# jakewendt/ghostm

Hardware: AMD Instinct MI355X
Metric: query residues aligned/sec (whole node) + bit-identical hit-list vs CPU (higher is better)
Workload: dtype int (exact 16-bit integers; packed f16 max3 orders their patterns, no guard)

## Files before the change

ghostm_amd/csrc/device.hip:

```cpp
#include <hip/hip_runtime.h>

#include <algorithm>
#include <atomic>
#include <climits>
#include <cstdio>
#include <cstdlib>
#include <cstring>
#include <mutex>
#include <string>
#include <vector>

#include "../../include/ghostm_hip.h"
#include "band_align.h"
#include "frame_align.h"
#include "common.h"
#include "device.h"
#include "formats.h"
#include "hit_batches.h"
#include "index.h"
#include "kernels.h"
#include "path_rows.h"
#include "read_rows.h"
#include "read_pileup.h"
#include "pileup_plan.h"
// ... 185 lines not shown
  DevBuf subj;
  DevBuf subj_bucket;
  uint32_t nsubj = 0;
};

struct DeviceModule::Impl {
  int h_matrix[32 * 32] = {0};
  static constexpr int kStageSlots = 4;
  static constexpr size_t kStagePiece = 8u << 20;
  PinnedBuf stage[kStageSlots];
  hipEvent_t stage_ev[kStageSlots] = {};
  bool stage_busy[kStageSlots] = {};
  int stage_turn = 0;
  DevBuf mat_k2, mat_tb, mat_tbk;
  DevBuf mat_raw;
  DevBuf counts, nelem, slots, offsets, qlist, gbuf, gbuf_off, list_beg, list_len;
  DevBuf cand_start, cand_qid;
  DevBuf records, rec_prefix;
  std::vector<uint32_t> h_rec_prefix;
  uint64_t ncand = 0;
  DevBuf task_buf[2], tasks_redo, score_out, end_out, guard_list;
  int task_turn = 0;
  struct Prepared {
    bool valid = false;
    uint64_t cand_begin = 0, n = 0;
    uint32_t count = 0, per_block = 0;
    bool swar = false;
    int kind = kScoreRows;
    int buf = 0;
  } prepared;
  struct ScoreState {
    bool active = false, guarded = false;
    uint64_t cand_begin = 0, n = 0;
    size_t lds = 0;
    int S = 32;
    kern::ScoreArgs args{};
  } score_state;
  struct DeferredNext {
    bool valid = false;
    DeviceModule::ScoreSegment seg{};
    bool swar = false, pairs_ok = true;
    uint32_t per_block = 0;
    size_t bytes = 0;
    uint32_t sparse_per_block = 0;
  } deferred;
  DevBuf tb_qid, tb_end, tb_start, tb_ml;
  DevBuf tb_ext;
  DevBuf tb_path_in, tb_path_meta, tb_path_dir, tb_path_ops, tb_path_cmp;
  DevBuf path_rows_hit, path_rows_ops, path_rows_out, path_rows_buf;
  DevBuf read_rows_hit, read_rows_ops, read_rows_out, read_rows_buf;
  DevBuf pileup_hit, pileup_ops, pileup_list, pileup_part, pileup_prof, pileup_out, pileup_cols;
  DevBuf band_hit, band_meta, band_dir, band_ops, band_cmp;
  DevBuf frame_hit, frame_meta, frame_dir, frame_ops, frame_cmp;
  DevBuf tb_width, tb_ncols, tb_skey, tb_key, tb_order1, tb_order2, tb_sort, tb_pair_a, tb_pair_b, tb_best;
  int cus = 256;
  DevBuf keys, sel_count, sel_score, sel_sid, slot_hits, sel_from;
  struct MergeState {
    bool active = false;
    uint32_t ng = 0;
// ... 57 lines not shown
  out->data = p;
  out->n = n;
}

DeviceModule &DeviceModule::Get() {
  static DeviceModule *m = new DeviceModule();
  return *m;
}

void DeviceModule::Use() const {
  thread_local int current = -1;
  if (device_ >= 0 && current != device_) {
    HIP_CHECK(hipSetDevice(device_));
    current = device_;
  }
}

void DeviceModule::Bind(int device) {
  if (device_ == device && impl_) {
    Use();
    return;
  }
  if (impl_ && device_ >= 0)
    throw Error("the device module is bound to device " + std::to_string(device_) + "; one device per process");
  int n = 0;
  HIP_CHECK(hipGetDeviceCount(&n));
  if (n <= 0) throw Error("no HIP device visible");
  if (device < 0 || device >= n) throw Error("device id " + std::to_string(device) + " out of range");
  HIP_CHECK(hipSetDevice(device));
  if (!impl_) impl_ = new Impl();
// ... 58 lines not shown
  HIP_CHECK(hipFuncSetAttribute((const void *)kern::k_tb_scan<SS, true, EE, true, true, true>, \
                                hipFuncAttributeMaxDynamicSharedMemorySize, (int)kScanLdsPriv));
  GHOSTM_SCAN_ATTRP(32, true) GHOSTM_SCAN_ATTRP(32, false) GHOSTM_SCAN_ATTRP(16, true)
  GHOSTM_SCAN_ATTRP(16, false) GHOSTM_SCAN_ATTRP(8, true) GHOSTM_SCAN_ATTRP(8, false)
#undef GHOSTM_SCAN_ATTRP
  for (const void *f : {(const void *)kern::k_score_pair<32>, (const void *)kern::k_score_pair<16>,
                        (const void *)kern::k_score_pair<8>})
    HIP_CHECK(hipFuncSetAttribute(f, hipFuncAttributeMaxDynamicSharedMemorySize, (int)(kern::kPairK2Words * 4)));
#undef GHOSTM_SCAN_ATTR2
#undef GHOSTM_SCAN_ATTR
  {
    hipDeviceProp_t p;
    HIP_CHECK(hipGetDeviceProperties(&p, device));
    impl_->cus = p.multiProcessorCount > 0 ? p.multiProcessorCount : 256;
  }
  device_ = device;
}

static hipStream_t S(void *s) { return static_cast<hipStream_t>(s); }

std::string DeviceModule::DeviceName() const {
  hipDeviceProp_t p;
  HIP_CHECK(hipGetDeviceProperties(&p, device_ < 0 ? 0 : device_));
  return std::string(p.name) + " (" + p.gcnArchName + ")";
}

size_t DeviceModule::TotalMemory() const {
  hipDeviceProp_t p;
  HIP_CHECK(hipGetDeviceProperties(&p, device_ < 0 ? 0 : device_));
  return p.totalGlobalMem;
// ... 21 lines not shown
        const int v = q == (int)kern::kPadCode ? -lim - 1 : std::max(-lim, std::min(lim, m[c * 32 + q]));
        tbk[w][c * 32 + q] =
            (int)(((uint32_t)v << (mlw + 2)) | (2u << mlw) | 0x80u | (c == q ? 1u : 0u));
      }
    }
  }
  impl_->mat_raw.Reserve(sizeof(impl_->h_matrix));
  HIP_CHECK(hipMemcpy(impl_->mat_raw.p, impl_->h_matrix, sizeof(impl_->h_matrix), hipMemcpyHostToDevice));
  impl_->mat_k2.Reserve(sizeof(k2));
  impl_->mat_tb.Reserve(sizeof(tb));
  impl_->mat_tbk.Reserve(sizeof(tbk));
  HIP_CHECK(hipMemcpy(impl_->mat_k2.p, k2, sizeof(k2), hipMemcpyHostToDevice));
  HIP_CHECK(hipMemcpy(impl_->mat_tb.p, tb, sizeof(tb), hipMemcpyHostToDevice));
  HIP_CHECK(hipMemcpy(impl_->mat_tbk.p, tbk, sizeof(tbk), hipMemcpyHostToDevice));
  impl_->matrix_set = true;
}

void DeviceModule::SetHostCopy(HostCopyFn fn) { host_copy_ = std::move(fn); }
void DeviceModule::SetHostParallel(HostParallelFn fn) { host_par_ = std::move(fn); }

void DeviceModule::StagedUpload(void *dst, const void *src, size_t bytes) {
  Impl &I = *impl_;
  if (bytes < (1u << 20) || !host_copy_) {
    if (bytes) HIP_CHECK(hipMemcpyAsync(dst, src, bytes, hipMemcpyHostToDevice, S(stream_)));
    if (bytes) HIP_CHECK(hipStreamSynchronize(S(stream_)));
    return;
  }
  for (size_t off = 0; off < bytes; off += Impl::kStagePiece) {
    const size_t n = std::min(Impl::kStagePiece, bytes - off);
    const int k = I.stage_turn;
// ... 822 lines not shown
  const bool framed = half && sigma_max <= 1000 && !(force && strcmp(force, "f16plain") == 0);
  const int64_t swar_low = 1024 + 64 + (-(int64_t)gap.open) + (-(int64_t)gap.ext);
  const int64_t swar_restart = swar_low + sigma_max + bound + 32;
  const int64_t swar_top = swar_restart + sigma_max + bound + std::abs((int64_t)gap.open - gap.ext) + 32;
  const bool swar = framed && swar_top < 0x7C00 && !(force && strcmp(force, "f16frame") == 0);
  const int64_t swar_rise = swar_top - swar_restart;
  const int64_t swar_step = swar_rise + 32;
  const uint64_t max_ends = d->end_gap == UINT32_MAX || base == 0 ? 1 : (uint64_t)(base - 1) / d->end_gap + 1;
  const int64_t swar_cap = swar_restart + (int64_t)(max_ends - 1) * swar_step;
  const char *levels_env = getenv("GHOSTM_K2_LEVELS");
  const bool levels = swar && !(levels_env && strcmp(levels_env, "0") == 0) && max_ends <= 64 && swar_cap + swar_rise < 0x7C00;
  int guard = swar ? 0 : framed ? (bound + sigma_max < 2040 ? 0 : (int)(2040 - sigma_max)) : (bound < 2048 ? 0 : 2000);
  if (half && getenv("GHOSTM_K2_GUARD")) guard = atoi(getenv("GHOSTM_K2_GUARD"));
  const uint32_t per_block = ScorePerBlock(q, d, base, gap);
  const uint32_t sparse_pb = swar ? SparsePerBlock(q, d) : 0u;
  int kind = kScoreRows;
  int buf = -1;
  size_t ntasks = 0;
  auto task_bytes = [&](uint64_t cn, uint32_t q0, uint32_t q1) {
    const uint32_t pb = sparse_pb ? std::min(per_block, sparse_pb) : per_block;
    return std::max<size_t>(ScoreTaskBound(cn, q0, q1, pb, kern::kScoreQmaxUnit) * sizeof(kern::ScoreTask),
                            (size_t)cn * 4);
  };
  if (I.prepared.valid && I.prepared.cand_begin == cand_begin && I.prepared.n == n &&
      I.prepared.per_block == per_block && I.prepared.swar == swar) {
    buf = I.prepared.buf;
    ntasks = I.prepared.count;
    kind = I.prepared.kind;
    HIP_CHECK(hipStreamWaitEvent(S(stream_), I.ev_tasks, 0));
  }
  const bool stale = I.prepared.valid;
  I.prepared.valid = false;
  if (buf < 0) {
    buf = I.task_turn;
    if (stale) HIP_CHECK(hipEventSynchronize(I.ev_tasks));
    PinnedBuf &hs = I.h_tasks[buf];
    hs.Reserve(task_bytes(n, q_first, q_end));
    ntasks = BuildTasks(swar, cand_begin, n, q_first, q_end, counts, offsets, per_block, hs.as<kern::ScoreTask>(),
                        &kind, guard == 0, &host_par_, sparse_pb);
    TraceMark("tasks", ntasks);
    if (const char *dump = getenv("GHOSTM_DEBUG_TASKS")) {
      if (FILE *f = fopen(dump, "ab")) {
        const uint64_t hdr[6] = {cand_begin, n, q_first, q_end, (uint64_t)kind, (uint64_t)ntasks};
        fwrite(hdr, 8, 6, f);
        fwrite(hs.p, kind == kScorePairs ? 4 : sizeof(kern::ScoreTask), ntasks, f);
        fwrite(counts.data() + q_first, 4, q_end - q_first, f);
        fwrite(offsets.data() + q_first, 8, q_end - q_first, f);
        fclose(f);
      }
    }
    const size_t tb = ntasks * (kind == kScorePairs ? 4 : sizeof(kern::ScoreTask));
    I.task_buf[buf].Reserve(tb);
    HIP_CHECK(hipMemcpyAsync(I.task_buf[buf].p, hs.p, tb, hipMemcpyHostToDevice, S(stream_)));
    TraceMark("tasks_up", ntasks);
// ... 28 lines not shown
  a.extend = gap.extend;
  a.open = gap.open;
  a.ext = gap.ext;
  a.score_out = I.score_out.as<uint32_t>();
  a.end_out = I.end_out.as<uint32_t>();
  a.out_base = cand_begin;
  a.swar_low = (uint32_t)swar_low;
  a.swar_restart = (uint32_t)swar_restart;
  a.swar_step = levels ? (uint32_t)swar_step : 0u;
  a.swar_cap = levels ? (uint32_t)swar_cap : 0u;
  if (pairs) {
    a.pairs = I.task_buf[buf].as<uint32_t>();
    a.npairs = (uint32_t)ntasks;
    a.fcodes = q->fcodes.as<uint32_t>();
  }
  if (sparse) {
    a.Lpad = slay.Lpad;
    a.pad = slay.Lpad - q->L;
    a.G = slay.G;
    a.gpw = slay.gpw;
    a.prof_slots = kern::SparseSlots();
    a.prof_rows = kern::kProfRowsSparse;
  }
  I.counters.Reserve(32);
  HIP_CHECK(hipMemsetAsync(I.counters.p, 0, 32, S(stream_)));
  a.cells = I.counters.as<unsigned long long>();
  if (half && guard) {
    I.guard_list.Reserve((size_t)n * 8);
    a.guard = guard;
    a.guard_count = reinterpret_cast<uint32_t *>(I.counters.as<unsigned long long>() + 2);
    a.guard_list = I.guard_list.as<uint32_t>();
  }
  const size_t lds = unit     ? (size_t)kern::kScoreQmaxUnit * kern::kProfRows16 * (lay.Lpad + 4) * 4 + 32 * 32 * 4
                     : sparse ? (size_t)kern::SparseSlots() * kern::kProfRowsSparse * (slay.Lpad + 8) * 2 + 32 * 32 * 2
                     : packed ? (size_t)kern::kScoreQmax * kern::kProfRows16 * (lay.Lpad + 8) * 2 + 32 * 32 * 2
                              : (size_t)kern::kScoreQmax * kern::kProfRows * (lay.Lpad + 4) * 4;
  HIP_CHECK(hipEventRecord(I.ev0, S(stream_)));
  const dim3 grid((uint32_t)ntasks), block(kern::kScoreBlock);
  if (pairs) {
    uint32_t ps = std::min<uint32_t>((uint32_t)lay.S, 16);
    if (const char *e = getenv("GHOSTM_K2_PAIR_S")) ps = (uint32_t)atoi(e);
    const uint32_t pg = ps == 8 || ps == 16 || ps == 32 ? lay.Lpad / ps : 0;
    const Layout play = pg >= 1 && pg <= 16 && pg * ps == lay.Lpad ? Layout{(int)ps, pg, lay.Lpad, 64 / pg} : lay;
    a.G = play.G;
    a.gpw = play.gpw;
    const uint32_t per_wg = (kern::kPairBlock / 64) * play.gpw;
    const dim3 pgrid(std::max<uint32_t>(1, std::min<uint32_t>((uint32_t)I.cus, (uint32_t)((ntasks + per_wg - 1) / per_wg))));
    const dim3 pblock(kern::kPairBlock);
// ... 49 lines not shown
  times_.score_launches_swar += swar ? 1 : 0;
  times_.score_launches_unit += unit ? 1 : 0;
  times_.score_launches_pair += pairs ? 1 : 0;
  times_.score_launches_sparse += sparse ? 1 : 0;
  times_.score_launches_levels += levels && (sparse || (packed && !unit && !pairs)) ? 1 : 0;
  P.active = true;
  P.guarded = half && guard;
  P.cand_begin = cand_begin;
  P.n = n;
  P.lds = lds;
  P.S = lay.S;
  P.args = a;
  I.deferred = Impl::DeferredNext{};
  if (next && next->n) {
    I.deferred = Impl::DeferredNext{true, *next, swar, guard == 0, per_block,
                                    task_bytes(next->n, next->q_first, next->q_end), sparse_pb};
    if (!defer_next_) ScorePrepareNext(counts, offsets);
  }
}

void DeviceModule::ScorePrepareNext(const std::vector<uint32_t> &counts, const std::vector<uint64_t> &offsets) {
  Impl &I = *impl_;
  if (!I.deferred.valid) return;
  const Impl::DeferredNext dn = I.deferred;
  I.deferred.valid = false;
  const ScoreSegment *next = &dn.seg;
  const int nb = I.task_turn;
  PinnedBuf &hs = I.h_tasks[nb];
  int nkind = kScoreRows;
  hs.Reserve(dn.bytes);
  const size_t nt = BuildTasks(dn.swar, next->cand_begin, next->n, next->q_first, next->q_end, counts, offsets,
                               dn.per_block, hs.as<kern::ScoreTask>(), &nkind, dn.pairs_ok, nullptr,
                               dn.sparse_per_block);
  const size_t nbytes = nt * (nkind == kScorePairs ? 4 : sizeof(kern::ScoreTask));
  I.task_buf[nb].Reserve(nbytes);
  HIP_CHECK(hipMemcpyAsync(I.task_buf[nb].p, hs.p, nbytes, hipMemcpyHostToDevice, S(copy_stream_)));
  HIP_CHECK(hipEventRecord(I.ev_tasks, S(copy_stream_)));
  I.prepared = Impl::Prepared{true, next->cand_begin, next->n, (uint32_t)nt, dn.per_block, dn.swar, nkind, nb};
}

bool DeviceModule::ScoreGuarded() const { return impl_ && impl_->score_state.active && impl_->score_state.guarded; }

void DeviceModule::ScoreFinish() {
  Use();
  Impl &I = *impl_;
  Impl::ScoreState &P = I.score_state;
  if (!P.active) return;
  P.active = false;
  SettleSeedTime();
  unsigned long long cells = 0;
  uint32_t nguard = 0;
  HIP_CHECK(hipStreamWaitEvent(S(copy_stream_), I.ev1, 0));
  HIP_CHECK(hipMemcpyAsync(&cells, I.counters.p, 8, hipMemcpyDeviceToHost, S(copy_stream_)));
// ... 1945 lines not shown
```

ghostm_amd/csrc/kernels.h:

```cpp
#pragma once
#include <hip/hip_runtime.h>
#include <stdint.h>

#include <type_traits>

#include "lds_poison.h"
#include "libstdcxx_sort.h"
#include "score_task.h"
#include "seed_lists.h"

namespace ghostm {
namespace kern {

constexpr uint32_t kSeqEnd = 25;
constexpr uint32_t kPadCode = 31;
constexpr int kNeg = -30000;

__device__ inline uint32_t ShiftUp(uint32_t v) {
  return (uint32_t)__builtin_amdgcn_mov_dpp((int)v, 0x138, 0xF, 0xF, true);
}

constexpr uint32_t kMaxLists = 128;
constexpr uint32_t kOverflow = 0xFFFFFFFFu;
#ifndef GHOSTM_K1_SLOT
// ... 1197 lines not shown
  uint32_t base, extend;
  int open, ext;
  uint32_t *score_out;
  uint32_t *end_out;
  unsigned long long out_base;
  unsigned long long *cells;
  int guard;
  uint32_t *guard_count;
  uint32_t *guard_list;
  uint32_t swar_low, swar_restart;
  const uint32_t *pairs;
  uint32_t npairs;
  const uint32_t *fcodes;
  uint32_t prof_slots, prof_rows;
  uint32_t swar_step, swar_cap;
};
__device__ inline uint32_t ProfSlots(const ScoreArgs &a) { return a.prof_slots ? a.prof_slots : (uint32_t)kScoreQmax; }
__device__ inline uint32_t ProfRows(const ScoreArgs &a) { return a.prof_rows ? a.prof_rows : kProfRows16; }

template <int S>
__global__ __launch_bounds__(kScoreBlock) void k_score(ScoreArgs a) {
  GHOSTM_POISON_LDS();
  extern __shared__ __attribute__((aligned(16))) int s_prof[];
  const ScoreTask t = a.tasks[blockIdx.x];
  const uint32_t RS = a.Lpad + 4;

  const uint32_t per_slot = kProfRows * a.Lpad;
  const uint32_t total = t.q_count * per_slot;
  for (uint32_t e = threadIdx.x; e < total; e += kScoreBlock) {
    const uint32_t slot = e / per_slot, rem = e - slot * per_slot;
// ... 246 lines not shown
#pragma unroll
      for (int k = 0; k < 4; ++k) {
        const uint4 v = src[k];
        w[4 * k] = v.x;
        w[4 * k + 1] = v.y;
        w[4 * k + 2] = v.z;
        w[4 * k + 3] = v.w;
      }
    }
#pragma unroll
    for (int c = 0; c < 32; ++c)
      if ((uint32_t)c < nrows) dst[c * RS] = (short)((c & 1) ? w[c >> 1] >> 16 : w[c >> 1]);
  }
}

__device__ __forceinline__ void BuildProfileUnit(const ScoreArgs &a, const ScoreTask &t, uint32_t *s_prof32,
                                                 uint32_t RS) {
  uint32_t *s_enc = s_prof32 + kScoreQmaxUnit * kProfRows16 * RS;
  const int extp = -a.ext;
  const uint32_t drop = (uint32_t)(0x10000u - (a.swar_low - 64u)) & 0xFFFFu;
  for (uint32_t e = threadIdx.x; e < 32 * 32; e += kScoreBlock) {
    const uint32_t q = e >> 5, c = e & 31;
    const int v = c < 25 ? a.mat[c * 32 + q] : 0;
    const uint32_t v16 = c < kSeqEnd ? (uint32_t)(v + extp) & 0xFFFFu : drop;
    s_enc[e] = v16 | 0x10000u;
  }
  __syncthreads();
  const uint32_t rows = t.q_count * a.Lpad;
  for (uint32_t p = threadIdx.x; p < rows; p += kScoreBlock) {
    const uint32_t slot = p / a.Lpad, r = p - slot * a.Lpad;
    uint32_t *dst = s_prof32 + slot * kProfRows16 * RS + r;
    if (r < a.pad) {
#pragma unroll
      for (int c = 0; c < 32; ++c) dst[c * RS] = drop | 0x10000u;
    } else {
      const uint32_t query = slot ? t.q_second : t.q_first;
      const uint32_t q = a.qseq[(size_t)query * a.L + (r - a.pad)];
      const uint4 *src = reinterpret_cast<const uint4 *>(s_enc + q * 32);
#pragma unroll
      for (int k = 0; k < 8; ++k) {
        const uint4 v = src[k];
        dst[(4 * k) * RS] = v.x;
        dst[(4 * k + 1) * RS] = v.y;
        dst[(4 * k + 2) * RS] = v.z;
        dst[(4 * k + 3) * RS] = v.w;
      }
    }
  }
}

template <int S, bool HALF>
__global__ __launch_bounds__(kScoreBlock) void k_score16(ScoreArgs a) {
  GHOSTM_POISON_LDS();
  using C = Cells<HALF>;
  extern __shared__ __attribute__((aligned(16))) short s_prof16[];
  const ScoreTask t = a.tasks[blockIdx.x];
  const uint32_t RS = a.Lpad + 8;

  BuildProfile16<C, false>(a, t, s_prof16, RS);
  __syncthreads();

// ... 134 lines not shown
                                             : 0ull);
}

#ifndef GHOSTM_K2_LAREUSE
#define GHOSTM_K2_LAREUSE 1
#endif
template <int S, bool SWAR = false, bool UNIT = false, bool LEVELS = false>
__global__ __launch_bounds__(kScoreBlock) void k_score16f(ScoreArgs a) {
  GHOSTM_POISON_LDS();
  static_assert(!UNIT || SWAR, "unit-pair words carry integer patterns");
  static_assert(!LEVELS || (SWAR && !UNIT), "restart levels: the 16-bit-row integer-pattern kernel");
  constexpr bool LA = UNIT || LEVELS;
  using C = Cells<true>;
  extern __shared__ __attribute__((aligned(16))) short s_prof16[];
  const ScoreTask t = a.tasks[blockIdx.x];
  const uint32_t RS = UNIT ? a.Lpad + 4 : a.Lpad + 8;
  const int extp = -a.ext;

  if constexpr (UNIT)
    BuildProfileUnit(a, t, reinterpret_cast<uint32_t *>(s_prof16), RS);
  else
    BuildProfile16<C, true, SWAR, LEVELS>(a, t, s_prof16, RS);
  __syncthreads();

  const uint32_t lane = threadIdx.x & 63, wave = threadIdx.x >> 6;
  const uint32_t g = lane / a.G, i = lane - g * a.G;
  const uint32_t pair = wave * a.gpw + g;
  const bool in_group = g < a.gpw;
  const bool vA = in_group && 2 * pair < t.count;
  const bool vB = in_group && 2 * pair + 1 < t.count;
  if (!__builtin_amdgcn_ballot_w64(vA)) return;
  unsigned long long cA = t.begin + 2 * pair, cB = cA + 1;
  uint32_t slotA = 0, slotB = 0, offA = 0, offB = 0, wA = 0, wB = 0;
  if constexpr (UNIT) {
    const uint32_t lA = 2 * pair, lB = lA + 1;
    slotA = vA && lA >= t.count1;
    slotB = vB && lB >= t.count1;
    cA = slotA ? t.begin2 + (lA - t.count1) : t.begin + lA;
    cB = slotB ? t.begin2 + (lB - t.count1) : t.begin + lB;
  }
  if (vA) {
    if constexpr (!UNIT) slotA = a.cand_qid[cA] - t.q_first;
    int o = (int)(a.cand_start[cA] - a.extend);
    offA = o < 0 ? 0u : (uint32_t)o;
    wA = a.base;
    if (offA + wA > a.dblen) wA = a.dblen - offA;
  }
  if (vB) {
    if constexpr (!UNIT) slotB = a.cand_qid[cB] - t.q_first;
    int o = (int)(a.cand_start[cB] - a.extend);
    offB = o < 0 ? 0u : (uint32_t)o;
    wB = a.base;
    if (offB + wB > a.dblen) wB = a.dblen - offB;
  }
  typedef unsigned int u32x4 __attribute__((ext_vector_type(4)));
  typedef __attribute__((address_space(3))) const u32x4 lds_u4;
  const uint32_t lds0 = (uint32_t)(uintptr_t)(__attribute__((address_space(3))) const char *)s_prof16;
  constexpr uint32_t EB = UNIT ? 4 : 2;
  const uint32_t SLOT = (UNIT ? kProfRows16 : ProfRows(a)) * RS;
  const uint32_t baseA2 = lds0 + (slotA * SLOT + i * S) * EB;
  const uint32_t baseB2 = lds0 + (slotB * SLOT + i * S) * EB;
  const uint8_t *dbp = a.db - kDbFrontPad;
  const uint32_t back = kDbFrontPad + a.dblen;
  const uint32_t xA = (vA ? offA + kDbFrontPad : back) - i, xB = (vB ? offB + kDbFrontPad : back) - i;
  const uint32_t RS2 = RS * EB;
  const __amdgpu_buffer_rsrc_t dbr = __builtin_amdgcn_make_buffer_rsrc((void *)dbp, 0, 0x7FFFFFFF, 0x00020000);
  const uint32_t EXTP = SWAR ? (uint32_t)extp * 0x10001u : C::Pair(extp);
  const hf2 KOE = HF(C::Pair(a.open - a.ext));
  const hf2 NEXT = HF(C::Pair(a.ext));
  const uint32_t KOE32 = (uint32_t)((a.open - a.ext) * 65537);
  const uint32_t NEXT32 = (uint32_t)(a.ext * 65537);
  const uint32_t ONE = SWAR ? 0x00010001u : C::kOne;
  const uint32_t RESTART = a.swar_restart * 0x10001u;
  const uint32_t SWLOW = a.swar_low * 0x10001u;
// ... 60 lines not shown
    } else {
      end = end_mask();
      any_end = __builtin_amdgcn_ballot_w64(end != 0) != 0;
    }
    const bool quiet = !tested && !any_end && (SWAR || !any_prev);
    any_prev = any_end;
    uint32_t sigc = sig;
    if constexpr (SWAR) {
      mreg = ONE;
      if (any_end && LEVELS) {
        sigc = BfiV(end, rlev, sig);
        rlev = PkMinU16(rlev + (end & STEP2), CAP2);
      } else if (any_end) {
        sigc = BfiV(end, RESTART, sig);
        mreg = ONE & ~end;
        const uint32_t reset = end & seen;
        seen |= end;
        if (__builtin_amdgcn_ballot_w64(reset != 0)) {
          if constexpr (UNIT) {
#pragma unroll
            for (int k = 0; k < S; ++k) {
              E[k] = BfiV(reset, RESTART, E[k]);
              H[k] = BfiV(reset, SWLOW, H[k]);
            }
            hprev = BfiV(reset, SWLOW, hprev);
          } else {
#pragma unroll
            for (int k = 0; k < S; ++k) E[k] = BfiV(reset, 0u, E[k]);
          }
        }
// ... 4 lines not shown
    hprev = hin;
    const hf2 m = HF(mreg);
    const uint32_t zn = SWAR ? sigc + EXTP : BfiV(end, EXTP, W(HF(sig) + HF(EXTP)));
    uint32_t zf = zn;
    if constexpr (LA) {
      la_any = __builtin_amdgcn_ballot_w64(max((uint16_t)c0A, (uint16_t)c0B) >= (uint16_t)kSeqEnd) != 0;
      la_ne = 0;
      if (la_any) {
        uint32_t ne = PkSign(PkAddU16(c0A | (c0B << 16), 0x7FE77FE7u));
        if constexpr (in_fill) ne = (int)(step - i) + 1 < 0 ? 0u : ne;
        la_ne = ne;
        zf = BfiV(ne, LEVELS ? rlev : RESTART, zn);
      }
    }
    const hf2 Z1 = HF(zf);
    lds_u4 *pA = (lds_u4 *)(uintptr_t)MadU24s(rA, RS2, baseA2);
    lds_u4 *pB = (lds_u4 *)(uintptr_t)MadU24s(rB, RS2, baseB2);
    uint32_t diag = diag0, F = fin, cm = sigc;
    auto diag_sum = [&](uint32_t h, uint32_t p) -> uint32_t {
      if constexpr (SWAR) return W(U2(h) * U2(mreg) + U2(p));
      else return C::Diag(h, m, p);
    };
#pragma unroll
    for (int k = 0; k < S; k += 8) {
      uint32_t wa[8], wb[8];
      if constexpr (UNIT) {
        const u32x4 qa0 = pA[k / 4], qa1 = pA[k / 4 + 1];
        const u32x4 qb0 = pB[k / 4], qb1 = pB[k / 4 + 1];
        wa[0] = qa0.x; wa[1] = qa0.y; wa[2] = qa0.z; wa[3] = qa0.w;
        wa[4] = qa1.x; wa[5] = qa1.y; wa[6] = qa1.z; wa[7] = qa1.w;
// ... 78 lines not shown
    if (obb > BB || (obb == BB && ocb > CB)) { BB = obb; CB = ocb; }
  }
  if (i == 0) {
    if (vA) {
      a.score_out[cA - a.out_base] = (uint32_t)BA;
      a.end_out[cA - a.out_base] = offA + (uint32_t)CA;
    }
    if (vB) {
      a.score_out[cB - a.out_base] = (uint32_t)BB;
      a.end_out[cB - a.out_base] = offB + (uint32_t)CB;
    }
    if (a.guard) {
      if (vA && BA >= a.guard) {
        const uint32_t k = atomicAdd(a.guard_count, 1u);
        a.guard_list[2 * k] = (uint32_t)(cA - a.out_base);
        a.guard_list[2 * k + 1] = UNIT ? (slotA ? t.q_second : t.q_first) : t.q_first + slotA;
      }
      if (vB && BB >= a.guard) {
        const uint32_t k = atomicAdd(a.guard_count, 1u);
        a.guard_list[2 * k] = (uint32_t)(cB - a.out_base);
        a.guard_list[2 * k + 1] = UNIT ? (slotB ? t.q_second : t.q_first) : t.q_first + slotB;
      }
    }
  }
  WaveAddCells(a.cells, (in_group && i == 0) ? (unsigned long long)((vA ? ncolsA : 0u) + (vB ? ncolsB : 0u)) * a.L
                                             : 0ull);
}

constexpr uint32_t kPairK2Codes = 27;
constexpr uint32_t kPairK2Stride = 33;
constexpr uint32_t kPairK2Words = kPairK2Codes * kPairK2Codes * kPairK2Stride;
constexpr uint32_t kPairPadCode = 25;
constexpr int kPairBlock = 768;
constexpr uint32_t kPairSingle = kPairSingleBit;

__global__ void k_fwd_codes(const uint8_t *qseq, uint32_t nq, uint32_t L, uint32_t Lpad, uint32_t *out) {
// ... 2578 lines not shown
```

ghostm_amd/csrc/score_task.h:

```cpp
#pragma once
#include <cstdint>
#include <cstdlib>

namespace ghostm {
namespace kern {

constexpr int kScoreQmax = 4;
constexpr int kScoreQmaxUnit = 2;
constexpr int kScoreQmaxSparse = 7;
inline uint32_t SparseSlots() {
  static const uint32_t v = [] {
    const char *e = getenv("GHOSTM_K2_SPARSE_SLOTS");
    const int k = e ? atoi(e) : kScoreQmaxSparse;
    return (uint32_t)(k >= 1 && k <= kScoreQmaxSparse ? k : kScoreQmaxSparse);
  }();
  return v;
}
constexpr uint32_t kProfRowsSparse = 27;
constexpr uint32_t kPairSingleBit = 0x80000000u;

struct ScoreTask {
  unsigned long long begin;
  uint32_t count;
  uint32_t q_first;
  uint32_t q_count;
  uint32_t count1;
  unsigned long long begin2;
  uint32_t q_second;
  uint32_t pad;
};

}
}
```

ghostm_amd/csrc/score_tasks.h:

```cpp
#pragma once
#include <algorithm>
#include <cstdint>
#include <cstdio>
#include <cstdlib>
#include <cstring>
#include <functional>
#include <utility>
#include <vector>

#include "score_task.h"


namespace ghostm {

using HostParallelFn = std::function<void(size_t parts, const std::function<void(size_t)> &fn)>;

inline size_t ScoreTaskBound(uint64_t n, uint32_t q_first, uint32_t q_end, uint32_t per_block, uint32_t qmax) {
  return (size_t)(n / per_block) + (q_end - q_first) + 2;
}
inline size_t BuildScoreTasks(uint64_t cand_begin, uint64_t n, uint32_t q_first, uint32_t q_end,
                              const std::vector<uint32_t> &counts, const std::vector<uint64_t> &offsets,
                              uint32_t per_block, uint32_t qmax, kern::ScoreTask *out) {
  size_t nt = 0;
  kern::ScoreTask cur{};
// ... 6 lines not shown
  for (uint32_t qi = q_first; qi < q_end; ++qi) {
    uint64_t lo = std::max<uint64_t>(offsets[qi], cand_begin);
    const uint64_t hi = std::min<uint64_t>(offsets[qi] + counts[qi], cand_end);
    while (lo < hi) {
      if (open_task && (cur.count == per_block || qi - cur.q_first >= qmax)) flush();
      if (!open_task) {
        cur = kern::ScoreTask{};
        cur.begin = lo;
        cur.q_first = qi;
        open_task = true;
      }
      const uint64_t take = std::min<uint64_t>(hi - lo, per_block - cur.count);
      cur.count += (uint32_t)take;
      cur.q_count = qi - cur.q_first + 1;
      if (qi == cur.q_first) cur.count1 += (uint32_t)take;
      cur.begin2 = cur.begin + cur.count1;
      cur.q_second = cur.q_first + 1;
      lo += take;
    }
  }
  flush();
  return nt;
}

inline size_t BuildScoreTasksPaired(uint64_t cand_begin, uint64_t n, uint32_t q_first, uint32_t q_end,
                                    const std::vector<uint32_t> &counts, const std::vector<uint64_t> &offsets,
                                    uint32_t per_block, kern::ScoreTask *out) {
  size_t nt = 0;
  auto single = [&](uint32_t q, uint64_t begin, uint32_t count) {
    kern::ScoreTask t{};
    t.begin = begin;
    t.count = count;
    t.count1 = count;
    t.q_first = q;
    t.q_count = 1;
    t.begin2 = begin + count;
    t.q_second = q;
    out[nt++] = t;
  };
  const uint64_t cand_end = cand_begin + n;
  std::vector<uint32_t> start(per_block + 1, 0);
  auto range = [&](uint32_t qi, uint64_t *lo, uint64_t *hi) {
    *lo = std::max<uint64_t>(offsets[qi], cand_begin);
    *hi = std::min<uint64_t>(offsets[qi] + counts[qi], cand_end);
  };
  for (uint32_t qi = q_first; qi < q_end; ++qi) {
    uint64_t lo, hi;
    range(qi, &lo, &hi);
    if (lo < hi && (hi - lo) % per_block) ++start[(hi - lo) % per_block + 1];
  }
  for (uint32_t r = 1; r <= per_block; ++r) start[r] += start[r - 1];
  std::vector<uint32_t> top(start.begin(), start.end() - 1);
// ... 12 lines not shown
    while (top[r1] > start[r1]) {
      const std::pair<uint32_t, uint64_t> a = rem[--top[r1]];
      uint32_t pick = 0;
      for (uint32_t r2 = std::min(r1, per_block - r1); r2 >= 1 && !pick; --r2)
        if (top[r2] > start[r2]) pick = r2;
      if (!pick) {
        single(a.first, a.second, r1);
        continue;
      }
      const std::pair<uint32_t, uint64_t> b = rem[--top[pick]];
      kern::ScoreTask t{};
      t.begin = a.second;
      t.count1 = r1;
      t.q_first = a.first;
      t.begin2 = b.second;
      t.q_second = b.first;
      t.count = r1 + pick;
      t.q_count = 2;
      out[nt++] = t;
    }
  }
  return nt;
}

inline size_t CountScoreTasks(uint64_t cand_begin, uint64_t n, uint32_t q_first, uint32_t q_end,
                              const std::vector<uint32_t> &counts, const std::vector<uint64_t> &offsets,
                              uint32_t per_block, uint32_t qmax) {
  size_t nt = 0;
  uint32_t cur = 0, open_q = 0;
  bool open_task = false;
  const uint64_t cand_end = cand_begin + n;
  for (uint32_t qi = q_first; qi < q_end; ++qi) {
// ... 70 lines not shown
  std::vector<uint64_t> rem(per_block, 0);
  size_t full = 0;
  const uint64_t cand_end = cand_begin + n;
  for (uint32_t qi = q_first; qi < q_end; ++qi) {
    const uint64_t lo = std::max<uint64_t>(offsets[qi], cand_begin);
    const uint64_t hi = std::min<uint64_t>(offsets[qi] + counts[qi], cand_end);
    if (lo >= hi) continue;
    full += (hi - lo) / per_block;
    ++rem[(hi - lo) % per_block];
  }
  return full + PairedFromRemainders(std::move(rem), per_block);
}

inline void CountTasks(uint64_t cand_begin, uint64_t n, uint32_t q_first, uint32_t q_end,
                       const std::vector<uint32_t> &counts, const std::vector<uint64_t> &offsets, uint32_t per_block,
                       size_t *n2, size_t *n4, size_t *np) {
  struct Runs {
    uint32_t qmax, cur = 0, open_q = 0;
    bool open = false;
    size_t nt = 0;
    void Add(uint32_t qi, uint64_t len, uint32_t per_block) {
      while (len) {
        if (open && (cur == per_block || qi - open_q >= qmax)) {
          ++nt;
          open = false;
        }
        if (!open) {
          cur = 0;
          open_q = qi;
          open = true;
        }
        const uint64_t take = std::min<uint64_t>(len, per_block - cur);
        cur += (uint32_t)take;
        len -= take;
      }
    }
    size_t Done() const { return nt + (open && cur ? 1 : 0); }
  } two{kern::kScoreQmaxUnit}, four{kern::kScoreQmax};
  std::vector<uint64_t> rem(per_block, 0);
  size_t full = 0;
  const uint64_t cand_end = cand_begin + n;
  for (uint32_t qi = q_first; qi < q_end; ++qi) {
    const uint64_t lo = std::max<uint64_t>(offsets[qi], cand_begin);
    const uint64_t hi = std::min<uint64_t>(offsets[qi] + counts[qi], cand_end);
    if (lo >= hi) continue;
    two.Add(qi, hi - lo, per_block);
    four.Add(qi, hi - lo, per_block);
    full += (hi - lo) / per_block;
    ++rem[(hi - lo) % per_block];
  }
  *n2 = two.Done();
  *n4 = four.Done();
  *np = full + PairedFromRemainders(rem, per_block);
// ... 31 lines not shown
  (*par)(parts, [&](size_t k) { write(cut(k), cut(k + 1), at[k]); });
  return at[parts];
}

enum ScoreKind { kScoreRows = 0, kScoreUnit = 1, kScorePairs = 2, kScoreRowsSparse = 3 };
constexpr uint64_t kScorePairMax = 16;

inline bool SparseRowsDefault() {
  const char *e = getenv("GHOSTM_K2_SPARSE");
  return !(e && strcmp(e, "pair") == 0);
}

inline size_t BuildTasks(bool swar, uint64_t cand_begin, uint64_t n, uint32_t q_first, uint32_t q_end,
                         const std::vector<uint32_t> &counts, const std::vector<uint64_t> &offsets,
                         uint32_t per_block, kern::ScoreTask *out, int *kind_out, bool pairs_ok = true,
                         const HostParallelFn *par = nullptr, uint32_t sparse_per_block = 0) {
  const char *k2 = getenv("GHOSTM_K2");
  const char *how = getenv("GHOSTM_K2_TASKS");
  const bool force_unit = k2 && strcmp(k2, "unit") == 0, force_rows = k2 && strcmp(k2, "swar16") == 0;
  const bool force_pair = k2 && strcmp(k2, "pair") == 0;
  const bool force_sparse = k2 && strcmp(k2, "sparse") == 0 && sparse_per_block;
  bool unit = false, paired = false;
  const uint64_t per_query = n / std::max<uint32_t>(1, q_end - q_first);
  uint64_t pair_max = kScorePairMax;
  if (const char *e = getenv("GHOSTM_K2_PAIR_MAX")) pair_max = strtoull(e, nullptr, 10);
  if (swar && q_end > q_first && (force_sparse || (!force_pair && sparse_per_block && pairs_ok && !force_unit &&
                                                    !force_rows && !how && per_query < pair_max &&
                                                    SparseRowsDefault()))) {
    *kind_out = kScoreRowsSparse;
    return BuildScoreTasksParallel(cand_begin, n, q_first, q_end, counts, offsets, sparse_per_block,
                                   kern::SparseSlots(), out, par);
  }
  if (swar && pairs_ok && q_end > q_first && !force_unit && !force_rows && !how &&
      (force_pair || per_query < pair_max)) {
    *kind_out = kScorePairs;
    return BuildScorePairs(cand_begin, n, q_first, q_end, counts, offsets, reinterpret_cast<uint32_t *>(out), par);
  }
  if (swar && q_end > q_first && !force_rows && !how && !force_unit && per_query >= 96) {
    unit = true;
  } else if (swar && q_end > q_first && !force_rows && (how || force_unit || per_query >= 24)) {
    size_t nc, n4, np;
    CountTasks(cand_begin, n, q_first, q_end, counts, offsets, per_block, &nc, &n4, &np);
    paired = how ? strcmp(how, "paired") == 0 : np * 100 <= nc * 95;
    const size_t nu = paired ? np : nc;
    unit = force_unit || nu * 100 <= n4 * 107;
    if (getenv("GHOSTM_DEBUG_TASKS"))
      fprintf(stderr, "k2 tasks: %llu candidates, %u queries: consecutive(2) %zu, paired %zu, consecutive(4) %zu -> %s\n",
              (unsigned long long)n, q_end - q_first, nc, np, n4, unit ? (paired ? "unit paired" : "unit consecutive") : "rows");
  }
  *kind_out = unit ? kScoreUnit : kScoreRows;
  if (unit && paired) return BuildScoreTasksPaired(cand_begin, n, q_first, q_end, counts, offsets, per_block, out);
  return BuildScoreTasksParallel(cand_begin, n, q_first, q_end, counts, offsets, per_block,
                                 unit ? kern::kScoreQmaxUnit : kern::kScoreQmax, out, par);
}

}
```

Measured before the change: 367.3 million.

## Allow three queries per unit score block and move substitution table to global

```diff
diff --git a/ghostm_amd/csrc/device.hip b/ghostm_amd/csrc/device.hip
--- a/ghostm_amd/csrc/device.hip
+++ b/ghostm_amd/csrc/device.hip
@@ -223,6 +223,11 @@
   int stage_turn = 0;
   DevBuf mat_k2, mat_tb, mat_tbk;
   DevBuf mat_raw;
+  DevBuf unit_tab;
+  bool unit_tab_valid = false;
+  int unit_tab_ext = 0;
+  uint32_t unit_tab_low = 0;
+  uint32_t unit_slots = kern::kScoreQmaxUnitMin;
   DevBuf counts, nelem, slots, offsets, qlist, gbuf, gbuf_off, list_beg, list_len;
   DevBuf cand_start, cand_qid;
   DevBuf records, rec_prefix;
@@ -237,6 +242,7 @@
     bool swar = false;
     int kind = kScoreRows;
     int buf = 0;
+    uint32_t unit_slots = 0;
   } prepared;
   struct ScoreState {
     bool active = false, guarded = false;
@@ -252,6 +258,7 @@
     uint32_t per_block = 0;
     size_t bytes = 0;
     uint32_t sparse_per_block = 0;
+    uint32_t unit_slots = kern::kScoreQmaxUnitMin;
   } deferred;
   DevBuf tb_qid, tb_end, tb_start, tb_ml;
   DevBuf tb_ext;
@@ -339,6 +346,10 @@
     HIP_CHECK(hipSetDevice(device_));
     current = device_;
   }
+}
+
+static size_t UnitLds(uint32_t slots, uint32_t Lpad) {
+  return ((size_t)slots * kern::kUnitRows + 1) * (Lpad + 4) * 4;
 }
 
 void DeviceModule::Bind(int device) {
@@ -427,6 +438,15 @@
     HIP_CHECK(hipGetDeviceProperties(&p, device));
     impl_->cus = p.multiProcessorCount > 0 ? p.multiProcessorCount : 256;
   }
+  {
+    int blocks = 0;
+    HIP_CHECK(hipOccupancyMaxActiveBlocksPerMultiprocessor(&blocks, (const void *)kern::k_score16f<32, true, true>,
+                                                           kern::kScoreBlock, UnitLds(kern::kScoreQmaxUnit, 128)));
+    impl_->unit_slots = blocks >= 4 ? kern::kScoreQmaxUnit : kern::kScoreQmaxUnitMin;
+    if (TraceOn() || getenv("GHOSTM_DEBUG_TASKS"))
+      fprintf(stderr, "k2 unit: %d blocks per CU at %zu bytes of LDS (three slots) -> %u slots per block\n", blocks,
+              UnitLds(kern::kScoreQmaxUnit, 128), impl_->unit_slots);
+  }
   device_ = device;
 }
 
@@ -478,6 +498,7 @@
   HIP_CHECK(hipMemcpy(impl_->mat_tb.p, tb, sizeof(tb), hipMemcpyHostToDevice));
   HIP_CHECK(hipMemcpy(impl_->mat_tbk.p, tbk, sizeof(tbk), hipMemcpyHostToDevice));
   impl_->matrix_set = true;
+  impl_->unit_tab_valid = false;
 }
 
 void DeviceModule::SetHostCopy(HostCopyFn fn) { host_copy_ = std::move(fn); }
@@ -1330,16 +1351,19 @@
   if (half && getenv("GHOSTM_K2_GUARD")) guard = atoi(getenv("GHOSTM_K2_GUARD"));
   const uint32_t per_block = ScorePerBlock(q, d, base, gap);
   const uint32_t sparse_pb = swar ? SparsePerBlock(q, d) : 0u;
+  uint32_t unit_slots = I.unit_slots;
+  if (const char *e = getenv("GHOSTM_K2_UNIT_SLOTS"))
+    if (atoi(e) == kern::kScoreQmaxUnit || atoi(e) == kern::kScoreQmaxUnitMin) unit_slots = (uint32_t)atoi(e);
   int kind = kScoreRows;
   int buf = -1;
   size_t ntasks = 0;
   auto task_bytes = [&](uint64_t cn, uint32_t q0, uint32_t q1) {
     const uint32_t pb = sparse_pb ? std::min(per_block, sparse_pb) : per_block;
-    return std::max<size_t>(ScoreTaskBound(cn, q0, q1, pb, kern::kScoreQmaxUnit) * sizeof(kern::ScoreTask),
+    return std::max<size_t>(ScoreTaskBound(cn, q0, q1, pb, unit_slots) * sizeof(kern::ScoreTask),
                             (size_t)cn * 4);
   };
   if (I.prepared.valid && I.prepared.cand_begin == cand_begin && I.prepared.n == n &&
-      I.prepared.per_block == per_block && I.prepared.swar == swar) {
+      I.prepared.per_block == per_block && I.prepared.swar == swar && I.prepared.unit_slots == unit_slots) {
     buf = I.prepared.buf;
     ntasks = I.prepared.count;
     kind = I.prepared.kind;
@@ -1353,7 +1377,7 @@
     PinnedBuf &hs = I.h_tasks[buf];
     hs.Reserve(task_bytes(n, q_first, q_end));
     ntasks = BuildTasks(swar, cand_begin, n, q_first, q_end, counts, offsets, per_block, hs.as<kern::ScoreTask>(),
-                        &kind, guard == 0, &host_par_, sparse_pb);
+                        &kind, guard == 0, &host_par_, sparse_pb, unit_slots);
     TraceMark("tasks", ntasks);
     if (const char *dump = getenv("GHOSTM_DEBUG_TASKS")) {
       if (FILE *f = fopen(dump, "ab")) {
@@ -1412,6 +1436,19 @@
     a.npairs = (uint32_t)ntasks;
     a.fcodes = q->fcodes.as<uint32_t>();
   }
+  if (unit) {
+    a.prof_slots = unit_slots;
+    if (!I.unit_tab_valid || I.unit_tab_ext != gap.ext || I.unit_tab_low != (uint32_t)swar_low) {
+      I.unit_tab.Reserve(32 * 32 * 4);
+      hipLaunchKernelGGL(kern::k_unit_table, dim3(4), dim3(256), 0, S(stream_), I.mat_k2.as<int>(), gap.ext,
+                         (uint32_t)swar_low, I.unit_tab.as<uint32_t>());
+      HIP_CHECK(hipGetLastError());
+      I.unit_tab_valid = true;
+      I.unit_tab_ext = gap.ext;
+      I.unit_tab_low = (uint32_t)swar_low;
+    }
+    a.unit_table = I.unit_tab.as<uint32_t>();
+  }
   if (sparse) {
     a.Lpad = slay.Lpad;
     a.pad = slay.Lpad - q->L;
@@ -1429,7 +1466,7 @@
     a.guard_count = reinterpret_cast<uint32_t *>(I.counters.as<unsigned long long>() + 2);
     a.guard_list = I.guard_list.as<uint32_t>();
   }
-  const size_t lds = unit     ? (size_t)kern::kScoreQmaxUnit * kern::kProfRows16 * (lay.Lpad + 4) * 4 + 32 * 32 * 4
+  const size_t lds = unit     ? UnitLds(unit_slots, lay.Lpad)
                      : sparse ? (size_t)kern::SparseSlots() * kern::kProfRowsSparse * (slay.Lpad + 8) * 2 + 32 * 32 * 2
                      : packed ? (size_t)kern::kScoreQmax * kern::kProfRows16 * (lay.Lpad + 8) * 2 + 32 * 32 * 2
                               : (size_t)kern::kScoreQmax * kern::kProfRows * (lay.Lpad + 4) * 4;
@@ -1509,7 +1546,7 @@
   I.deferred = Impl::DeferredNext{};
   if (next && next->n) {
     I.deferred = Impl::DeferredNext{true, *next, swar, guard == 0, per_block,
-                                    task_bytes(next->n, next->q_first, next->q_end), sparse_pb};
+                                    task_bytes(next->n, next->q_first, next->q_end), sparse_pb, unit_slots};
     if (!defer_next_) ScorePrepareNext(counts, offsets);
   }
 }
@@ -1526,12 +1563,13 @@
   hs.Reserve(dn.bytes);
   const size_t nt = BuildTasks(dn.swar, next->cand_begin, next->n, next->q_first, next->q_end, counts, offsets,
                                dn.per_block, hs.as<kern::ScoreTask>(), &nkind, dn.pairs_ok, nullptr,
-                               dn.sparse_per_block);
+                               dn.sparse_per_block, dn.unit_slots);
   const size_t nbytes = nt * (nkind == kScorePairs ? 4 : sizeof(kern::ScoreTask));
   I.task_buf[nb].Reserve(nbytes);
   HIP_CHECK(hipMemcpyAsync(I.task_buf[nb].p, hs.p, nbytes, hipMemcpyHostToDevice, S(copy_stream_)));
   HIP_CHECK(hipEventRecord(I.ev_tasks, S(copy_stream_)));
-  I.prepared = Impl::Prepared{true, next->cand_begin, next->n, (uint32_t)nt, dn.per_block, dn.swar, nkind, nb};
+  I.prepared = Impl::Prepared{true, next->cand_begin, next->n, (uint32_t)nt, dn.per_block, dn.swar, nkind, nb,
+                              dn.unit_slots};
 }
 
 bool DeviceModule::ScoreGuarded() const { return impl_ && impl_->score_state.active && impl_->score_state.guarded; }
diff --git a/ghostm_amd/csrc/kernels.h b/ghostm_amd/csrc/kernels.h
--- a/ghostm_amd/csrc/kernels.h
+++ b/ghostm_amd/csrc/kernels.h
@@ -1235,6 +1235,7 @@
   const uint32_t *fcodes;
   uint32_t prof_slots, prof_rows;
   uint32_t swar_step, swar_cap;
+  const uint32_t *unit_table;
 };
 __device__ inline uint32_t ProfSlots(const ScoreArgs &a) { return a.prof_slots ? a.prof_slots : (uint32_t)kScoreQmax; }
 __device__ inline uint32_t ProfRows(const ScoreArgs &a) { return a.prof_rows ? a.prof_rows : kProfRows16; }
@@ -1511,37 +1512,42 @@
   }
 }
 
+__global__ void k_unit_table(const int *mat, int ext, uint32_t swar_low, uint32_t *table) {
+  const uint32_t e = blockIdx.x * blockDim.x + threadIdx.x;
+  if (e >= 32 * 32) return;
+  const uint32_t q = e >> 5, c = e & 31;
+  const uint32_t drop = (uint32_t)(0x10000u - (swar_low - 64u)) & 0xFFFFu;
+  const int v = c < kSeqEnd ? mat[c * 32 + q] : 0;
+  const uint32_t v16 = c < kSeqEnd ? (uint32_t)(v - ext) & 0xFFFFu : drop;
+  table[e] = v16 | 0x10000u;
+}
+
 __device__ __forceinline__ void BuildProfileUnit(const ScoreArgs &a, const ScoreTask &t, uint32_t *s_prof32,
                                                  uint32_t RS) {
-  uint32_t *s_enc = s_prof32 + kScoreQmaxUnit * kProfRows16 * RS;
-  const int extp = -a.ext;
-  const uint32_t drop = (uint32_t)(0x10000u - (a.swar_low - 64u)) & 0xFFFFu;
-  for (uint32_t e = threadIdx.x; e < 32 * 32; e += kScoreBlock) {
-    const uint32_t q = e >> 5, c = e & 31;
-    const int v = c < 25 ? a.mat[c * 32 + q] : 0;
-    const uint32_t v16 = c < kSeqEnd ? (uint32_t)(v + extp) & 0xFFFFu : drop;
-    s_enc[e] = v16 | 0x10000u;
-  }
-  __syncthreads();
+  const uint32_t dropw = ((uint32_t)(0x10000u - (a.swar_low - 64u)) & 0xFFFFu) | 0x10000u;
+  uint32_t *shared_row = s_prof32 + a.prof_slots * kUnitRows * RS;
+  for (uint32_t r = threadIdx.x; r < a.Lpad; r += kScoreBlock) shared_row[r] = dropw;
   const uint32_t rows = t.q_count * a.Lpad;
+  const uint32_t q0 = t.q_first, q1 = t.q_second, q2 = t.q_third;
   for (uint32_t p = threadIdx.x; p < rows; p += kScoreBlock) {
     const uint32_t slot = p / a.Lpad, r = p - slot * a.Lpad;
-    uint32_t *dst = s_prof32 + slot * kProfRows16 * RS + r;
+    uint32_t *dst = s_prof32 + slot * kUnitRows * RS + r;
     if (r < a.pad) {
 #pragma unroll
-      for (int c = 0; c < 32; ++c) dst[c * RS] = drop | 0x10000u;
+      for (int c = 0; c < (int)kUnitRows; ++c) dst[c * RS] = dropw;
     } else {
-      const uint32_t query = slot ? t.q_second : t.q_first;
+      const uint32_t query = slot == 0 ? q0 : slot == 1 ? q1 : q2;
       const uint32_t q = a.qseq[(size_t)query * a.L + (r - a.pad)];
-      const uint4 *src = reinterpret_cast<const uint4 *>(s_enc + q * 32);
-#pragma unroll
-      for (int k = 0; k < 8; ++k) {
+      const uint4 *src = reinterpret_cast<const uint4 *>(a.unit_table + q * 32);
+#pragma unroll
+      for (int k = 0; k < 6; ++k) {
         const uint4 v = src[k];
         dst[(4 * k) * RS] = v.x;
         dst[(4 * k + 1) * RS] = v.y;
         dst[(4 * k + 2) * RS] = v.z;
         dst[(4 * k + 3) * RS] = v.w;
       }
+      dst[24 * RS] = a.unit_table[q * 32 + 24];
     }
   }
 }
@@ -1706,6 +1712,7 @@
   using C = Cells<true>;
   extern __shared__ __attribute__((aligned(16))) short s_prof16[];
   const ScoreTask t = a.tasks[blockIdx.x];
+  const uint32_t tq0 = t.q_first, tq1 = t.q_second, tq2 = t.q_third;
   const uint32_t RS = UNIT ? a.Lpad + 4 : a.Lpad + 8;
   const int extp = -a.ext;
 
@@ -1725,11 +1732,12 @@
   unsigned long long cA = t.begin + 2 * pair, cB = cA + 1;
   uint32_t slotA = 0, slotB = 0, offA = 0, offB = 0, wA = 0, wB = 0;
   if constexpr (UNIT) {
-    const uint32_t lA = 2 * pair, lB = lA + 1;
-    slotA = vA && lA >= t.count1;
-    slotB = vB && lB >= t.count1;
-    cA = slotA ? t.begin2 + (lA - t.count1) : t.begin + lA;
-    cB = slotB ? t.begin2 + (lB - t.count1) : t.begin + lB;
+    const uint32_t lA = 2 * pair, lB = lA + 1, c1 = t.count1, c12 = t.count1 + t.count2;
+    const unsigned long long b1 = t.begin, b2 = t.begin2 - c1, b3 = t.begin3 - c12;
+    slotA = vA ? (uint32_t)(lA >= c1) + (uint32_t)(lA >= c12) : 0u;
+    slotB = vB ? (uint32_t)(lB >= c1) + (uint32_t)(lB >= c12) : 0u;
+    cA = (slotA == 0 ? b1 : slotA == 1 ? b2 : b3) + lA;
+    cB = (slotB == 0 ? b1 : slotB == 1 ? b2 : b3) + lB;
   }
   if (vA) {
     if constexpr (!UNIT) slotA = a.cand_qid[cA] - t.q_first;
@@ -1749,7 +1757,9 @@
   typedef __attribute__((address_space(3))) const u32x4 lds_u4;
   const uint32_t lds0 = (uint32_t)(uintptr_t)(__attribute__((address_space(3))) const char *)s_prof16;
   constexpr uint32_t EB = UNIT ? 4 : 2;
-  const uint32_t SLOT = (UNIT ? kProfRows16 : ProfRows(a)) * RS;
+  const uint32_t SLOT = (UNIT ? kUnitRows : ProfRows(a)) * RS;
+  const uint32_t shA = UNIT ? kUnitRows * (a.prof_slots - slotA) : 0u;
+  const uint32_t shB = UNIT ? kUnitRows * (a.prof_slots - slotB) : 0u;
   const uint32_t baseA2 = lds0 + (slotA * SLOT + i * S) * EB;
   const uint32_t baseB2 = lds0 + (slotB * SLOT + i * S) * EB;
   const uint8_t *dbp = a.db - kDbFrontPad;
@@ -1840,6 +1850,11 @@
       } else if (any_end) {
         sigc = BfiV(end, RESTART, sig);
         mreg = ONE & ~end;
+        if constexpr (UNIT && !tested) {
+          rA = rA >= kSeqEnd ? shA : rA;
+          rB = rB >= kSeqEnd ? shB : rB;
+          asm volatile("" : "+v"(rA), "+v"(rB));
+        }
         const uint32_t reset = end & seen;
         seen |= end;
         if (__builtin_amdgcn_ballot_w64(reset != 0)) {
@@ -1874,6 +1889,10 @@
       }
     }
     const hf2 Z1 = HF(zf);
+    if constexpr (UNIT && tested) {
+      rA = rA >= kSeqEnd ? shA : rA;
+      rB = rB >= kSeqEnd ? shB : rB;
+    }
     lds_u4 *pA = (lds_u4 *)(uintptr_t)MadU24s(rA, RS2, baseA2);
     lds_u4 *pB = (lds_u4 *)(uintptr_t)MadU24s(rB, RS2, baseB2);
     uint32_t diag = diag0, F = fin, cm = sigc;
@@ -1982,12 +2001,12 @@
       if (vA && BA >= a.guard) {
         const uint32_t k = atomicAdd(a.guard_count, 1u);
         a.guard_list[2 * k] = (uint32_t)(cA - a.out_base);
-        a.guard_list[2 * k + 1] = UNIT ? (slotA ? t.q_second : t.q_first) : t.q_first + slotA;
+        a.guard_list[2 * k + 1] = UNIT ? (slotA == 0 ? tq0 : slotA == 1 ? tq1 : tq2) : tq0 + slotA;
       }
       if (vB && BB >= a.guard) {
         const uint32_t k = atomicAdd(a.guard_count, 1u);
         a.guard_list[2 * k] = (uint32_t)(cB - a.out_base);
-        a.guard_list[2 * k + 1] = UNIT ? (slotB ? t.q_second : t.q_first) : t.q_first + slotB;
+        a.guard_list[2 * k + 1] = UNIT ? (slotB == 0 ? tq0 : slotB == 1 ? tq1 : tq2) : tq0 + slotB;
       }
     }
   }
diff --git a/ghostm_amd/csrc/score_task.h b/ghostm_amd/csrc/score_task.h
--- a/ghostm_amd/csrc/score_task.h
+++ b/ghostm_amd/csrc/score_task.h
@@ -6,7 +6,9 @@
 namespace kern {
 
 constexpr int kScoreQmax = 4;
-constexpr int kScoreQmaxUnit = 2;
+constexpr int kScoreQmaxUnit = 3;
+constexpr int kScoreQmaxUnitMin = 2;
+constexpr uint32_t kUnitRows = 25;
 constexpr int kScoreQmaxSparse = 7;
 inline uint32_t SparseSlots() {
   static const uint32_t v = [] {
@@ -27,6 +29,9 @@
   uint32_t count1;
   unsigned long long begin2;
   uint32_t q_second;
+  uint32_t count2;
+  unsigned long long begin3;
+  uint32_t q_third;
   uint32_t pad;
 };
 
diff --git a/ghostm_amd/csrc/score_tasks.h b/ghostm_amd/csrc/score_tasks.h
--- a/ghostm_amd/csrc/score_tasks.h
+++ b/ghostm_amd/csrc/score_tasks.h
@@ -44,8 +44,11 @@
       cur.count += (uint32_t)take;
       cur.q_count = qi - cur.q_first + 1;
       if (qi == cur.q_first) cur.count1 += (uint32_t)take;
+      if (qi == cur.q_first + 1) cur.count2 += (uint32_t)take;
       cur.begin2 = cur.begin + cur.count1;
       cur.q_second = cur.q_first + 1;
+      cur.begin3 = cur.begin2 + cur.count2;
+      cur.q_third = cur.q_first + 2;
       lo += take;
     }
   }
@@ -64,8 +67,8 @@
     t.count1 = count;
     t.q_first = q;
     t.q_count = 1;
-    t.begin2 = begin + count;
-    t.q_second = q;
+    t.begin2 = t.begin3 = begin + count;
+    t.q_second = t.q_third = q;
     out[nt++] = t;
   };
   const uint64_t cand_end = cand_begin + n;
@@ -108,8 +111,10 @@
       t.count1 = r1;
       t.q_first = a.first;
       t.begin2 = b.second;
-      t.q_second = b.first;
+      t.q_second = t.q_third = b.first;
       t.count = r1 + pick;
+      t.count2 = pick;
+      t.begin3 = b.second + pick;
       t.q_count = 2;
       out[nt++] = t;
     }
@@ -210,7 +215,7 @@
 
 inline void CountTasks(uint64_t cand_begin, uint64_t n, uint32_t q_first, uint32_t q_end,
                        const std::vector<uint32_t> &counts, const std::vector<uint64_t> &offsets, uint32_t per_block,
-                       size_t *n2, size_t *n4, size_t *np) {
+                       size_t *n2, size_t *n4, size_t *np, uint32_t unit_qmax = kern::kScoreQmaxUnitMin) {
   struct Runs {
     uint32_t qmax, cur = 0, open_q = 0;
     bool open = false;
@@ -232,7 +237,7 @@
       }
     }
     size_t Done() const { return nt + (open && cur ? 1 : 0); }
-  } two{kern::kScoreQmaxUnit}, four{kern::kScoreQmax};
+  } two{unit_qmax}, four{kern::kScoreQmax};
   std::vector<uint64_t> rem(per_block, 0);
   size_t full = 0;
   const uint64_t cand_end = cand_begin + n;
@@ -294,7 +299,8 @@
 inline size_t BuildTasks(bool swar, uint64_t cand_begin, uint64_t n, uint32_t q_first, uint32_t q_end,
                          const std::vector<uint32_t> &counts, const std::vector<uint64_t> &offsets,
                          uint32_t per_block, kern::ScoreTask *out, int *kind_out, bool pairs_ok = true,
-                         const HostParallelFn *par = nullptr, uint32_t sparse_per_block = 0) {
+                         const HostParallelFn *par = nullptr, uint32_t sparse_per_block = 0,
+                         uint32_t unit_qmax = kern::kScoreQmaxUnitMin) {
   const char *k2 = getenv("GHOSTM_K2");
   const char *how = getenv("GHOSTM_K2_TASKS");
   const bool force_unit = k2 && strcmp(k2, "unit") == 0, force_rows = k2 && strcmp(k2, "swar16") == 0;
@@ -320,18 +326,31 @@
     unit = true;
   } else if (swar && q_end > q_first && !force_rows && (how || force_unit || per_query >= 24)) {
     size_t nc, n4, np;
-    CountTasks(cand_begin, n, q_first, q_end, counts, offsets, per_block, &nc, &n4, &np);
+    CountTasks(cand_begin, n, q_first, q_end, counts, offsets, per_block, &nc, &n4, &np, unit_qmax);
     paired = how ? strcmp(how, "paired") == 0 : np * 100 <= nc * 95;
     const size_t nu = paired ? np : nc;
     unit = force_unit || nu * 100 <= n4 * 107;
     if (getenv("GHOSTM_DEBUG_TASKS"))
-      fprintf(stderr, "k2 tasks: %llu candidates, %u queries: consecutive(2) %zu, paired %zu, consecutive(4) %zu -> %s\n",
-              (unsigned long long)n, q_end - q_first, nc, np, n4, unit ? (paired ? "unit paired" : "unit consecutive") : "rows");
+      fprintf(stderr, "k2 tasks: %llu candidates, %u queries: consecutive(%u) %zu, paired %zu, consecutive(4) %zu -> %s\n",
+              (unsigned long long)n, q_end - q_first, unit_qmax, nc, np, n4,
+              unit ? (paired ? "unit paired" : "unit consecutive") : "rows");
   }
   *kind_out = unit ? kScoreUnit : kScoreRows;
-  if (unit && paired) return BuildScoreTasksPaired(cand_begin, n, q_first, q_end, counts, offsets, per_block, out);
-  return BuildScoreTasksParallel(cand_begin, n, q_first, q_end, counts, offsets, per_block,
-                                 unit ? kern::kScoreQmaxUnit : kern::kScoreQmax, out, par);
-}
-
-}
+  const uint32_t qmax = unit ? unit_qmax : kern::kScoreQmax;
+  const size_t nt = unit && paired
+                        ? BuildScoreTasksPaired(cand_begin, n, q_first, q_end, counts, offsets, per_block, out)
+                        : BuildScoreTasksParallel(cand_begin, n, q_first, q_end, counts, offsets, per_block, qmax, out, par);
+  if (getenv("GHOSTM_DEBUG_TASKS") && nt) {
+    const size_t c2 = CountScoreTasks(cand_begin, n, q_first, q_end, counts, offsets, per_block, 2);
+    const size_t c3 = CountScoreTasks(cand_begin, n, q_first, q_end, counts, offsets, per_block, 3);
+    fprintf(stderr,
+            "k2 fill: %s(%u), %llu candidates, %u queries, %zu tasks x %u = %.4f; consecutive(2) %zu = %.4f, "
+            "consecutive(3) %zu = %.4f\n",
+            unit ? (paired ? "unit paired" : "unit consecutive") : "rows", paired ? 2u : qmax, (unsigned long long)n,
+            q_end - q_first, nt, per_block, (double)n / ((double)nt * per_block), c2,
+            (double)n / ((double)c2 * per_block), c3, (double)n / ((double)c3 * per_block));
+  }
+  return nt;
+}
+
+}
```

Result: slower. 358.8 million (-2.3%).
